# xuanvinh1997/llm-fp8

Hardware: AMD Instinct MI355X
Metric: train tokens/sec + FP8 GEMM % of MFMA peak, Llama-3.2-3B seq512 b16 (higher is better)
Workload: dtype fp8 (E4M3/E5M2 operands, fp32 accumulate, bf16 activations); 1 GPU; llama-3.2-3b (28 layers) full fine-tuning step, batch 16/GPU x seq 512, fp8_scenario=default (te_llama counterpart, lm_head FP8 under the outer recipe), random-init weights, synthetic tokens; route=fused, global_batch=16, seq_len=512, parallelism=single

## Files before the change

include/mi_fp8.h:

```cpp
#ifndef MI_FP8_H
#define MI_FP8_H

#include <stdint.h>

#ifdef __cplusplus
extern "C" {
#endif

#define MI_FMT_E4M3 0
#define MI_FMT_E5M2 1

#define MI_OK 0
#define MI_ERR_ARG (-1)
#define MI_ERR_SHAPE (-2)
#define MI_ERR_HIP (-3)

#define MI_OUT_BF16 0
#define MI_OUT_F32 1

#define MI_AMAX_ALGO_MAX 0
#define MI_AMAX_ALGO_MOST_RECENT 1

#define MI_ABI_VERSION 5
int mi_abi_version(void);
// ... 73 lines not shown

int mi_dswiglu_cast(const void* h_bf16, const void* dact_bf16, void* y_fp8, void* yT_fp8, const float* scale,
                    float* amax, float* colsum, int64_t rows, int64_t F, int fmt, void* stream);
int mi_swiglu_cast_bias(const void* h_bf16, const void* bias_bf16, void* y_fp8, void* yT_fp8, const float* scale, float* amax,
                        int64_t rows, int64_t F, int fmt, void* stream);
int mi_dswiglu_cast_bias(const void* h_bf16, const void* bias_bf16, const void* dact_bf16, void* y_fp8, void* yT_fp8,
                         const float* scale, float* amax, float* colsum, int64_t rows, int64_t F, int fmt, void* stream);

int mi_rmsnorm_stats(const void* x_bf16, float* rstd, int64_t rows, int64_t cols, float eps, void* stream);
int mi_add_rmsnorm_stats(const void* a_bf16, const void* b_bf16, void* out_bf16, float* rstd, int64_t rows, int64_t cols,
                         float eps, void* stream);
int mi_add_bias_rmsnorm_stats(const void* a_bf16, const void* b_bf16, const void* bias_bf16, void* out_bf16, float* rstd,
                              int64_t rows, int64_t cols, float eps, void* stream);
int mi_norm_cast(const void* x_bf16, const float* rstd, const void* gamma_bf16, void* y_fp8, void* yT_fp8,
                 const float* scale, float* amax, int64_t rows, int64_t cols, int fmt, void* stream);
int mi_rmsnorm_bwd(const void* dy_bf16, const void* x_bf16, const float* rstd, const void* gamma_bf16,
                   const void* dres_bf16, void* dx_bf16, float* dgamma_partial, int n_partials, int64_t rows,
                   int64_t cols, void* stream);

int mi_ce_forward(const void* logits_bf16, const int64_t* labels, float* lse, float* loss_rows, int64_t rows,
                  int64_t cols, void* stream);
int mi_ce_backward(const void* logits_bf16, const int64_t* labels, const float* lse, const float* gscale,
                   void* dlogits_bf16, int64_t rows, int64_t cols, void* stream);
int mi_ce_backward_cast(const void* logits_bf16, const int64_t* labels, const float* lse, const float* gscale, void* y_fp8,
                        void* yT_fp8, const float* scale, float* amax, int64_t rows, int64_t cols, int fmt, void* stream);

int mi_sumsq_bf16(const void* g_bf16, int64_t n, float* partial, int n_partials, void* stream);
int mi_sumsq_bf16_multi(const int64_t* table, int n_tensors, const int32_t* chunks, int n_chunks, int chunk_elems,
                        double* partial, void* stream);
int mi_adamw_bf16_multi(const int64_t* table, int n_tensors, const int32_t* chunks, int n_chunks, int chunk_elems,
// ... 31 lines not shown
```

llm_fp8_amd/_lib.py:

```python
from __future__ import annotations

import ctypes
import os

_HERE = os.path.dirname(os.path.abspath(__file__))
LIB_PATH = os.environ.get("LLM_FP8_AMD_LIB") or os.path.join(_HERE, "libmi_fp8.so")
LAB_LIB_PATH = os.path.join(os.path.dirname(_HERE), "tools", "bin", "libmi_fp8_lab.so")

MI_FMT_E4M3 = 0
MI_FMT_E5M2 = 1
ABI_VERSION = 5

_c_i64 = ctypes.c_int64
_c_int = ctypes.c_int
_p = ctypes.c_void_p

class GemmProblem(ctypes.Structure):
    _fields_ = [("A", ctypes.c_void_p), ("B", ctypes.c_void_p), ("D", ctypes.c_void_p), ("sa_inv", ctypes.c_void_p),
                ("sb_inv", ctypes.c_void_p), ("M", ctypes.c_int64), ("N", ctypes.c_int64), ("K", ctypes.c_int64),
                ("lda", ctypes.c_int64), ("ldb", ctypes.c_int64), ("ldd", ctypes.c_int64)]


class GemmMxProblem(ctypes.Structure):
    _fields_ = [("A", ctypes.c_void_p), ("SA", ctypes.c_void_p), ("B", ctypes.c_void_p), ("SB", ctypes.c_void_p),
# ... 38 lines not shown
    "mi_cast_amax_colsum": [_p, _p, _p, _p, _p, _p, _c_i64, _c_i64, _c_i64, _c_i64, _c_int, _p],
    "mi_colsum_finish": [_p, _c_i64, _c_i64, _p, _c_int, _p],
    "mi_colsum_finish_multi": [_p, _p, _p, _p, _p, _c_int, _p],
    "mi_gemm_workspace_bytes": [],
    "mi_gemm_set_workspace": [_p, _c_i64],
    "mi_attn_fwd": [_p, _p, _p, _p, _p, _c_int, _c_int, _c_int, _c_int, _c_int, _c_i64, _c_i64, _c_i64, _c_i64, ctypes.c_float,
                    _c_int, _p],
    "mi_attn_bwd": [_p] * 10 + [_c_int] * 5 + [_c_i64] * 8 + [ctypes.c_float, _c_int, _p],
    "mi_mxfp8_norm_quantize": [_p, _p, _p, _p, _p, _p, _p, _c_i64, _c_i64, _c_int, _p],
    "mi_mxfp8_swiglu_quantize": [_p, _p, _p, _p, _p, _c_i64, _c_i64, _c_int, _p],
    "mi_mxfp8_dswiglu_quantize": [_p, _p, _p, _p, _p, _p, _p, _c_i64, _c_i64, _c_int, _p],
    "mi_gemm_mxfp8": [_p, _p, _p, _p, _p, _p, _c_i64, _c_i64, _c_i64, _c_int, _c_int, _c_int, _c_int, _p],
    "mi_swiglu_cast_bias": [_p, _p, _p, _p, _p, _p, _c_i64, _c_i64, _c_int, _p],
    "mi_dswiglu_cast_bias": [_p, _p, _p, _p, _p, _p, _p, _p, _c_i64, _c_i64, _c_int, _p],
    "mi_add_bias_rmsnorm_stats": [_p, _p, _p, _p, _p, _c_i64, _c_i64, ctypes.c_float, _p],
    "mi_gemm_fp8_clock": [_p, _p, _p, _p, _p, _c_i64, _c_i64, _c_i64, _c_i64, _c_i64, _c_i64, _c_int, _p, _p],
}
LAB_SIGNATURES = {
    "mi_attn_fwd_diag": [_p, _p, _p, _p, _p, _p, _c_int, _c_int, _c_int, _c_int, _c_int, _c_i64, _c_i64, _c_i64, _c_i64, ctypes.c_float, _p],
}

_lib = None


def _bind(path: str, signatures) -> ctypes.CDLL:
    lib = ctypes.CDLL(path)
    for name, argtypes in signatures.items():
        fn = getattr(lib, name)
        fn.argtypes = argtypes
        fn.restype = ctypes.c_char_p if name == "mi_last_error" else (_c_i64 if name == "mi_gemm_workspace_bytes" else _c_int)
# ... 37 lines not shown
```

llm_fp8_amd/csrc/mi_fused.hip:

```cpp
#include "mi_common.h"

namespace mi {

template <int DIR>
__global__ __launch_bounds__(256) void rope_qkv_kernel(uint16_t* __restrict__ fused, uint16_t* __restrict__ q,
                                                       uint16_t* __restrict__ k, uint16_t* __restrict__ v,
                                                       const float* __restrict__ cosT, const float* __restrict__ sinT,
                                                       int rows, int seq, int nq, int nk, int D) {
  const int half = D >> 1;
  const int vph = half >> 3;
  const int W = (nq + 2 * nk) * D;
  const int rot_items = (nq + nk) * vph;
  const int cpy_items = (nk * D) >> 3;
  const int per_row = rot_items + cpy_items;
  const int64_t items = (int64_t)rows * per_row;
  const float sgn = DIR == 0 ? 1.0f : -1.0f;
  for (int64_t it = (int64_t)blockIdx.x * blockDim.x + threadIdx.x; it < items; it += (int64_t)gridDim.x * blockDim.x) {
    const int64_t r = it / per_row;
    const int w = (int)(it - r * per_row);
    uint16_t* frow = fused + r * W;
    if (w < rot_items) {
      const int hd = w / vph, vv = w - hd * vph;
      uint16_t* sep = hd < nq ? q + (r * nq + hd) * D : k + (r * nk + (hd - nq)) * D;
      uint16_t* f1 = frow + hd * D + vv * 8;
// ... 854 lines not shown
  const uint16_t *xp = (const uint16_t*)x_bf16, *gp = (const uint16_t*)gamma_bf16;
  uint8_t *yp = (uint8_t*)y_fp8, *tp = (uint8_t*)yT_fp8;
#define MI_NC(FMTv)                                                                                                        \
  if (y_fp8 && yT_fp8)                                                                                                     \
    hipLaunchKernelGGL((mi::norm_cast_kernel<FMTv, true, true>), grid, block, 0, st, xp, rstd, gp, yp, tp, scale, amax, (int)rows, (int)cols, tiles_c); \
  else if (y_fp8)                                                                                                          \
    hipLaunchKernelGGL((mi::norm_cast_kernel<FMTv, true, false>), grid, block, 0, st, xp, rstd, gp, yp, tp, scale, amax, (int)rows, (int)cols, tiles_c); \
  else                                                                                                                     \
    hipLaunchKernelGGL((mi::norm_cast_kernel<FMTv, false, true>), grid, block, 0, st, xp, rstd, gp, yp, tp, scale, amax, (int)rows, (int)cols, tiles_c);
  if (fmt == MI_FMT_E4M3) { MI_NC(MI_FMT_E4M3) } else { MI_NC(MI_FMT_E5M2) }
#undef MI_NC
  MI_CHECK_LAUNCH("mi_norm_cast launch");
  return MI_OK;
}

extern "C" int mi_rmsnorm_bwd(const void* dy_bf16, const void* x_bf16, const float* rstd, const void* gamma_bf16,
                              const void* dres_bf16, void* dx_bf16, float* dgamma_partial, int n_partials, int64_t rows,
                              int64_t cols, void* stream) {
  MI_CHECK_ARG(dy_bf16 && x_bf16 && rstd && gamma_bf16 && dx_bf16 && dgamma_partial, "mi_rmsnorm_bwd: null pointer");
  MI_CHECK_ARG(rows >= 0 && cols > 0 && cols % 512 == 0 && cols <= 512 * mi::kNormMaxVec, "mi_rmsnorm_bwd: cols must be a multiple of 512, at most %d", 512 * mi::kNormMaxVec);
  MI_CHECK_ARG(n_partials >= 1 && rows < (1LL << 31), "mi_rmsnorm_bwd: bad sizes");
  MI_CHECK_ARG(((uintptr_t)dy_bf16 % 16) == 0 && ((uintptr_t)x_bf16 % 16) == 0 && ((uintptr_t)gamma_bf16 % 16) == 0 &&
                   ((uintptr_t)dres_bf16 % 16) == 0 && ((uintptr_t)dx_bf16 % 16) == 0, "mi_rmsnorm_bwd: misaligned pointer");
  const int rows_per_block = (int)((rows + n_partials - 1) / n_partials);
  const int rpb = rows_per_block < 1 ? 1 : rows_per_block;
  const size_t shm = (size_t)(4 * cols * sizeof(float));
#define MI_RB(NV, WPRv)                                                                                                   \
  case NV:                                                                                                                \
    hipLaunchKernelGGL((mi::rmsnorm_bwd_kernel<NV, WPRv>), dim3(n_partials), dim3(256), shm, (hipStream_t)stream,         \
                       (const uint16_t*)dy_bf16, (const uint16_t*)x_bf16, rstd, (const uint16_t*)gamma_bf16,              \
// ... 67 lines not shown
```

llm_fp8_amd/llama.py:

```python
from __future__ import annotations

import os
import re
from contextlib import contextmanager
from typing import Dict, Optional

import torch

from . import pytorch as te
from .common.recipe import DelayedScaling, Format, MXFP8BlockScaling
from .pytorch.fp8 import FP8GlobalStateManager
from .pytorch.module import _can_fuse_norm, residual_add_stats

LLAMA_CONFIGS: Dict[str, dict] = {
    "llama-3.2-1b": dict(hidden_size=2048, intermediate_size=8192, num_hidden_layers=16, num_attention_heads=32,
                         num_key_value_heads=8, head_dim=64, tie_word_embeddings=True),
    "llama-3.2-3b": dict(hidden_size=3072, intermediate_size=8192, num_hidden_layers=28, num_attention_heads=24,
                         num_key_value_heads=8, head_dim=128, tie_word_embeddings=True),
    "llama-3.1-8b": dict(hidden_size=4096, intermediate_size=14336, num_hidden_layers=32, num_attention_heads=32,
                         num_key_value_heads=8, head_dim=128, tie_word_embeddings=False),
}
_ALIASES = {"meta-llama/llama-3.2-1b": "llama-3.2-1b", "meta-llama/llama-3.2-3b": "llama-3.2-3b",
            "meta-llama/llama-3.1-8b": "llama-3.1-8b", "meta-llama/meta-llama-3.1-8b": "llama-3.1-8b"}


def llama_config(name: str, **overrides):
    from transformers import LlamaConfig
# ... 26 lines not shown

_ROPE_CACHE: Dict[tuple, torch.Tensor] = {}


def _rope_table(dim: int, max_len: int, device) -> torch.Tensor:
    key = (dim, max_len, str(device))
    if key not in _ROPE_CACHE:
        _ROPE_CACHE[key] = te.attention.RotaryPositionEmbedding(dim)(max_seq_len=max_len).to(device)
    return _ROPE_CACHE[key]


def _handed_rstd(h: torch.Tensor):
    tag = getattr(h, "_mi_rstd", None)
    if tag is None or tag[2] != h._version:
        return None
    return tag[0], tag[1]


class TELlamaDecoderLayer(torch.nn.Module):

    scenario = "default"

    def __init__(self, config, *args, dropout_rate: float = 0.0, **kwargs):
        super().__init__()
        dev = "cuda" if torch.cuda.is_available() else "cpu"
        self.attn_recipe, self.mlp_recipe = scenario_recipes(self.scenario)
        self.self_attention = te.MultiheadAttention(
            hidden_size=config.hidden_size,
            num_attention_heads=config.num_attention_heads,
            kv_channels=getattr(config, "head_dim", None) or config.hidden_size // config.num_attention_heads,
            bias=False,
# ... 3 lines not shown
            normalization="RMSNorm",
            num_gqa_groups=config.num_key_value_heads,
            qkv_format="bshd",
            input_layernorm=True,
            device=dev,
        )
        self.layernorm_mlp = te.LayerNormMLP(
            hidden_size=config.hidden_size,
            ffn_hidden_size=config.intermediate_size,
            normalization="RMSNorm",
            activation="swiglu",
            device=dev,
        )
        head_dim = getattr(config, "head_dim", None) or config.hidden_size // config.num_attention_heads
        self.te_rope_emb = _rope_table(head_dim, config.max_position_embeddings, dev)

    route = "fused"

    def forward(self, hidden_states, attention_mask=None, **kwargs):
        if not isinstance(hidden_states, torch.Tensor):
            raise TypeError("hidden_states must be a torch.Tensor")
        if attention_mask is not None and not isinstance(attention_mask, torch.Tensor):
            raise TypeError("attention_mask must be a torch.Tensor")
        fp8 = hidden_states.is_cuda
        if self.route == "reference":
            with te.fp8_autocast(enabled=fp8, fp8_recipe=self.attn_recipe):
                hidden_states = hidden_states + self.self_attention(hidden_states, attention_mask=attention_mask,
                                                                    rotary_pos_emb=self.te_rope_emb)
            with te.fp8_autocast(enabled=fp8, fp8_recipe=self.mlp_recipe):
                hidden_states = hidden_states + self.layernorm_mlp(hidden_states)
            return hidden_states
        with te.fp8_autocast(enabled=fp8, fp8_recipe=self.attn_recipe):
            attn_out, skip = self.self_attention(hidden_states, attention_mask=attention_mask, rotary_pos_emb=self.te_rope_emb,
                                                 _with_skip=True, _rstd=_handed_rstd(hidden_states))
        eps_mlp = self.layernorm_mlp.eps
        hidden_states, rstd = residual_add_stats(skip, attn_out, eps_mlp)
        with te.fp8_autocast(enabled=fp8, fp8_recipe=self.mlp_recipe):
            ffn_out, skip, ffn_bias = self.layernorm_mlp(hidden_states, _with_skip=True, _rstd=(rstd, eps_mlp), _defer_bias=True)
        eps_in = self.self_attention.layernorm_qkv.eps
        hidden_states, rstd = residual_add_stats(skip, ffn_out, eps_in, bias=ffn_bias)
        if rstd is not None:
            hidden_states._mi_rstd = (rstd, eps_in, hidden_states._version)
        return hidden_states


def decoder_layer_cls(scenario: str):
    scenario_recipes(scenario)
    return type(f"TELlamaDecoderLayer_{scenario}", (TELlamaDecoderLayer,), {"scenario": scenario})


@contextmanager
def replace_decoder(te_decoder_cls):
    import transformers
    mod = transformers.models.llama.modeling_llama
    original = mod.LlamaDecoderLayer
    mod.LlamaDecoderLayer = te_decoder_cls
    try:
# ... 49 lines not shown

    model.forward = forward


class _FinalNormView:
    fused_norm, normalization, zero_centered_gamma = True, "RMSNorm", False


class TELlamaForCausalLM:

    def __new__(cls, config, scenario: str = "default"):
        from transformers.models.llama.modeling_llama import LlamaForCausalLM
        with replace_decoder(te_decoder_cls=decoder_layer_cls(scenario)):
            model = LlamaForCausalLM(config)
        model.model.register_forward_pre_hook(_drop_padding_mask, with_kwargs=True)
        _install_final_norm_fusion(model)
        return model

    @classmethod
    def from_pretrained_local(cls, pretrained_model_name_or_path, *args, config, scenario: str = "default",
                              torch_dtype=torch.bfloat16, **kwargs):
        from . import checkpoint
        prev = torch.get_default_dtype()
        torch.set_default_dtype(torch_dtype)
        try:
            model = cls(config, scenario)
        finally:
            torch.set_default_dtype(prev)
        checkpoint.load_into(model, str(pretrained_model_name_or_path), config)
        return model
# ... 122 lines not shown
```

llm_fp8_amd/pytorch/module.py:

```python
from __future__ import annotations

import io
import os
from typing import List, Optional, Sequence, Tuple

import torch
import torch.nn.functional as F

from ..common.recipe import DelayedScaling, Format, MXFP8BlockScaling, Recipe, fmt_codes
from . import ops
from .fp8 import FP8GlobalStateManager, ModuleMeta

__all__ = ["Linear", "LayerNormLinear", "LayerNormMLP", "LayerNorm", "RMSNorm"]


def _as_bf16_2d(t: torch.Tensor) -> torch.Tensor:
    t2 = t.reshape(-1, t.shape[-1])
    if t2.dtype != torch.bfloat16:
        t2 = t2.to(torch.bfloat16)
    return t2.contiguous()


class DyHandoff:
    __slots__ = ("scale", "amax", "fmt", "want_y", "want_t", "fp8", "ptr", "mx", "act_ref")
# ... 21 lines not shown
                               "(an op was inserted between the q|k|v projection and the rotary split)")
        fp8, self.fp8, self.ptr = self.fp8, None, None
        return fp8


def handoff_readers(t) -> bool:
    if torch.is_anomaly_enabled():
        return True
    if t is None:
        return False
    return bool(getattr(t, "retains_grad", False)) or bool(getattr(t, "_backward_hooks", None))


class _GemmSpec:
    __slots__ = ("recipe", "meta_fwd", "meta_bwd", "g", "fmt_fwd", "fmt_bwd", "trigger_bwd_update", "training", "eps",
                 "wcache", "first_mb", "with_skip", "rstd", "dy_handoff", "defer_bias", "q")

    def __init__(self, recipe, meta_fwd, meta_bwd, g, trigger_bwd_update, training, eps=1e-5, wcache=None, first_mb=None,
                 with_skip=False, rstd=None, dy_handoff=None, defer_bias=False):
        self.dy_handoff = dy_handoff
        self.defer_bias = defer_bias
        self.eps = eps
        self.rstd = rstd
        self.with_skip = with_skip
        self.wcache, self.first_mb = wcache, first_mb
        self.recipe, self.meta_fwd, self.meta_bwd, self.g = recipe, meta_fwd, meta_bwd, g
        self.fmt_fwd, self.fmt_bwd = fmt_codes(recipe.fp8_format)
        self.q = _MXQ(self.fmt_fwd, self.fmt_bwd) if recipe.mxfp8() else _DelayedQ(meta_fwd, meta_bwd, self.fmt_fwd, self.fmt_bwd)
        self.trigger_bwd_update = trigger_bwd_update
        self.training = training


class _Sink:
    __slots__ = ("parts", "stamp")

# ... 93 lines not shown
    no_sink = "row-sharded weights of this shape cannot take an FP8 sink"
    swiglu_adds_bias = True
    colsum_dtypes = None

    def __init__(self, mf, mb, fmt_f: int, fmt_b: int):
        self.mf, self.mb, self.fmt_f, self.fmt_b = mf, mb, fmt_f, fmt_b

    def _act(self, y, yT, s: int):
        return (y, self.mf.scale_inv(s)), (yT, self.mf.scale_inv_snapshot()[s:s + 1])

    def quantize(self, x2, g: int, want_t: bool, norm=None):
        mf, s = self.mf, 3 * g
        if norm is None:
            return self._act(*ops.cast_amax(x2, mf.scale(s), mf.amax(s), self.fmt_f, want_t=want_t), s)
        return self._act(*ops.norm_cast(x2, norm[0], norm[1], mf.scale(s), mf.amax(s), self.fmt_f, want_t=want_t), s)

    def swiglu(self, h, g: int, want_t: bool, bias):
        mf, s = self.mf, 3 * g
        return self._act(*ops.swiglu_cast(h, mf.scale(s), mf.amax(s), self.fmt_f, want_t=want_t, bias=bias), s)

    def _grad(self, y, yT, cs, s: int):
        si = self.mb.scale_inv(s)
        return (y, si), (yT, si), cs

    def quantize_grad(self, g2, g: int, want_y: bool, want_t: bool, colsum: bool = False):
        mb, s = self.mb, 2 * g
        out = ops.cast_amax(g2, mb.scale(s), mb.amax(s), self.fmt_b, want_y=want_y, want_t=want_t, want_colsum=colsum)
        return self._grad(out[0], out[1], out[2] if colsum else None, s)

    def dswiglu(self, h, dact, g: int, want_y: bool, want_t: bool, colsum: bool, bias):
# ... 165 lines not shown
    @staticmethod
    def backward(ctx, dout, _drstd):
        return dout, dout, None, None


def residual_add_stats(a: torch.Tensor, b: torch.Tensor, eps: float, bias: Optional[torch.Tensor] = None):
    if (a.is_cuda and a.dtype == torch.bfloat16 and b.dtype == torch.bfloat16 and a.shape == b.shape and a.is_contiguous()
            and b.is_contiguous() and a.shape[-1] % 8 == 0 and (bias is None or a.shape[-1] == bias.numel())):
        bb = None if bias is None else bias.detach().to(torch.bfloat16).contiguous()
        return _AddStatsFn.apply(a, b, eps, bb)
    if bias is not None:
        b = b + bias.detach().to(b.dtype)
    return a + b, None


def _wgrad_out(weights, K: int) -> Optional[torch.Tensor]:
    shard = getattr(weights[0], "_mi_sharded", None)
    if shard is not None:
        return shard.dp.wgrad_buffer(weights, K)
    slot = getattr(weights[0], "_mi_grad_slot", None)
    if slot is None:
        return None
    arena, off = slot
    if arena.dtype != torch.bfloat16:
        return None
    end = off
    for w in weights:
        s = getattr(w, "_mi_grad_slot", None)
        if s is None or s[0] is not arena or s[1] != end or w.grad is not None or w.dtype != torch.bfloat16 or w.shape[1] != K:
            return None
# ... 26 lines not shown
def _skip_2d(dskip: Optional[torch.Tensor], like: torch.Tensor) -> Optional[torch.Tensor]:
    if dskip is None:
        return None
    d = dskip.reshape(like.shape)
    return d if (d.dtype == torch.bfloat16 and d.is_contiguous()) else d.to(torch.bfloat16).contiguous()


def _quantize_input(ctx, spec: _GemmSpec, x2, ln_w, want_t: bool, need_dgrad: bool):
    ctx.norm = None
    if ln_w is None:
        return spec.q.quantize(x2, spec.g, want_t)
    gam = (ln_w if ln_w.dtype == torch.bfloat16 else ln_w.to(torch.bfloat16)).contiguous()
    rstd = spec.rstd if spec.rstd is not None else ops.rmsnorm_stats(x2, spec.eps)
    if need_dgrad:
        ctx.norm = (x2, rstd, gam, ln_w.dtype)
    return spec.q.quantize(x2, spec.g, want_t, (rstd, gam))


def _finish_dx(ctx, dx, dskip, colsums=None):
    dln = None
    if ctx.norm is not None and dx is not None:
        xin, rstd, gam, ln_dtype = ctx.norm
        ctx.norm = None
        dx, dln = ops.rmsnorm_bwd(dx, xin, rstd, gam, dres=_skip_2d(dskip, dx), dgamma_dtype=ln_dtype, finish=colsums is None)
        dskip = None
        if colsums is not None:
            dln = (dln, ln_dtype)
    if colsums is not None:
        pend = [t for t in (*colsums, dln) if t is not None]
        if pend:
# ... 298 lines not shown
        for n, sz in zip(self.bias_names, sizes):
            if bias:
                setattr(self, n, torch.nn.Parameter(torch.zeros(sz, dtype=dt, device=device)))
            else:
                setattr(self, n, None)

    def _weights(self):
        return [getattr(self, n) for n in self.weight_names]

    def _bias(self):
        if not self.use_bias:
            return None
        bs = [getattr(self, n) for n in self.bias_names]
        return bs[0] if len(bs) == 1 else torch.cat(bs, 0)

    def forward(self, inp: torch.Tensor, is_first_microbatch=None, _with_skip: bool = False, _rstd=None, _dy_handoff=None):
        st = self._prepare(inp.device)
        ws, b = self._weights(), self._bias()
        if st is not None and _can_fuse_norm(self, st[0], inp) and not self.return_layernorm_output:
            return _FP8LinearFn.apply(inp, b, self._spec(st, is_first_microbatch, eps=self.eps, with_skip=_with_skip,
                                                         rstd=_usable_rstd(_rstd, inp, self.eps), dy_handoff=_dy_handoff),
                                      self.layer_norm_weight, *ws)
        ln = self._norm(inp)
        if st is None:
            w = _master(ws[0]) if len(ws) == 1 else torch.cat([_master(w_) for w_ in ws], 0)
            out = F.linear(ln, w.to(ln.dtype), None if b is None else b.to(ln.dtype))
        else:
            out = _FP8LinearFn.apply(ln, b, self._spec(st, is_first_microbatch), None, *ws)
        if _with_skip:
            return out, inp
        return (out, ln) if self.return_layernorm_output else out


def _usable_rstd(handoff, inp: torch.Tensor, eps: float):
    if handoff is None:
        return None
    rstd, e = handoff
    if rstd is None or e != eps or rstd.numel() != inp.numel() // inp.shape[-1] or rstd.device != inp.device:
        return None
    return rstd


def _can_fuse_norm(mod, recipe, inp) -> bool:
    h = inp.shape[-1]
    return (getattr(mod, "fused_norm", True) and mod.normalization == "RMSNorm" and not mod.zero_centered_gamma
            and (recipe.delayed() or recipe.mxfp8()) and h % 512 == 0 and h // 512 in (1, 2, 3, 4, 5, 6, 7, 8, 10, 12, 14, 16))


def _swiglu(a: torch.Tensor) -> torch.Tensor:
    f = a.shape[-1] // 2
    return F.silu(a[..., :f]) * a[..., f:]


_ACTS = {
    "swiglu": (_swiglu, 2), "gelu": (lambda a: F.gelu(a, approximate="tanh"), 1), "relu": (F.relu, 1),
# ... 14 lines not shown
        self.hidden_size, self.ffn_hidden_size, self.eps = hidden_size, ffn_hidden_size, eps
        self.normalization, self.activation, self.zero_centered_gamma = normalization, activation, zero_centered_gamma
        self.act_fn, mult = _ACTS[activation]
        dt = params_dtype or torch.get_default_dtype()
        self.layer_norm_weight = torch.nn.Parameter(
            torch.zeros(hidden_size, dtype=dt, device=device) if zero_centered_gamma else torch.ones(hidden_size, dtype=dt, device=device))
        self.layer_norm_bias = (torch.nn.Parameter(torch.zeros(hidden_size, dtype=dt, device=device))
                                if normalization == "LayerNorm" else None)
        self.fc1_weight = _init_weight((mult * ffn_hidden_size, hidden_size), dt, device, init_method)
        self.fc2_weight = _init_weight((hidden_size, ffn_hidden_size), dt, device, output_layer_init_method or init_method)
        self.use_bias = bias
        self.fc1_bias = torch.nn.Parameter(torch.zeros(mult * ffn_hidden_size, dtype=dt, device=device)) if bias else None
        self.fc2_bias = torch.nn.Parameter(torch.zeros(hidden_size, dtype=dt, device=device)) if bias else None
        self.fused_swiglu = True

    def forward(self, inp: torch.Tensor, is_first_microbatch=None, _with_skip: bool = False, _rstd=None, _defer_bias: bool = False):
        st = self._prepare(inp.device)
        if (st is not None and self.activation == "swiglu" and self.fused_swiglu and _can_fuse_norm(self, st[0], inp)):
            defer = bool(_defer_bias and _with_skip and _FUSE_MLP_BIAS and self.fc2_bias is not None)
            res = _FP8SwiGLUMLPFn.apply(inp, self.fc1_weight, self.fc1_bias, self.fc2_weight, self.fc2_bias,
                                        self._spec(st, is_first_microbatch, eps=self.eps, with_skip=_with_skip,
                                                   rstd=_usable_rstd(_rstd, inp, self.eps), defer_bias=defer),
                                        self.layer_norm_weight)
            if _defer_bias and _with_skip:
                return res[0], res[1], (self.fc2_bias if defer else None)
            return res
        out = self._unfused(inp, st, is_first_microbatch)
        if _defer_bias and _with_skip:
            return out, inp, None
        return (out, inp) if _with_skip else out

    def _unfused(self, inp, st, is_first_microbatch):
        ln = self._norm(inp)
        if st is None:
            h = F.linear(ln, _master(self.fc1_weight).to(ln.dtype), None if self.fc1_bias is None else self.fc1_bias.to(ln.dtype))
            return F.linear(self.act_fn(h), _master(self.fc2_weight).to(ln.dtype),
                            None if self.fc2_bias is None else self.fc2_bias.to(ln.dtype))
# ... 7 lines not shown
```

llm_fp8_amd/pytorch/ops.py:

```python
from __future__ import annotations

import ctypes
import os
from typing import Optional, Tuple

import torch

from .. import _lib
from .profiler import KernelTimer

E4M3, E5M2 = _lib.MI_FMT_E4M3, _lib.MI_FMT_E5M2
FP8_MAX = {E4M3: 448.0, E5M2: 57344.0}


_SK_WORKSPACE = {}


def ensure_gemm_workspace(device: torch.device) -> None:
    idx = device.index if device.index is not None else torch.cuda.current_device()
    if idx in _SK_WORKSPACE:
        return
    lib = _lib.load()
    with torch.cuda.device(idx):
        nbytes = int(lib.mi_gemm_workspace_bytes())
# ... 575 lines not shown
    assert x.dtype == torch.bfloat16 and gamma.dtype == torch.bfloat16 and x.is_contiguous() and gamma.is_contiguous()
    R, C = x.shape
    y = torch.empty((R, C), dtype=torch.uint8, device=x.device) if want_y else None
    yT = torch.empty((C, R), dtype=torch.uint8, device=x.device) if want_t else None
    args = (x.data_ptr(), rstd.data_ptr(), gamma.data_ptr(), _ptr(y), _ptr(yT), scale.data_ptr(), _ptr(amax), R, C, fmt, _stream())
    t = KernelTimer.active
    if t is None:
        rc = _lib.load().mi_norm_cast(*args)
    else:
        with t.span("norm_cast", f"{R}x{C}", float(R * C), float(R * C * (2 + int(want_y) + int(want_t)))):
            rc = _lib.load().mi_norm_cast(*args)
    _lib.check(rc, "mi_norm_cast")
    return y, yT


def rmsnorm_bwd(dy: torch.Tensor, x: torch.Tensor, rstd: torch.Tensor, gamma: torch.Tensor,
                dres: Optional[torch.Tensor] = None, n_partials: int = 512, dgamma_dtype: torch.dtype = torch.float32,
                finish: bool = True):
    _dev(dy, x, rstd, gamma, dres)
    assert dy.dtype == torch.bfloat16 and x.dtype == torch.bfloat16 and dy.is_contiguous() and x.is_contiguous()
    R, C = x.shape
    n_partials = max(1, min(n_partials, (R + 3) // 4))
    dx = torch.empty_like(x)
    part = torch.empty((n_partials, C), dtype=torch.float32, device=x.device)
    rc = _lib.load().mi_rmsnorm_bwd(dy.data_ptr(), x.data_ptr(), rstd.data_ptr(), gamma.data_ptr(), _ptr(dres), dx.data_ptr(),
                                    part.data_ptr(), n_partials, R, C, _stream())
    _lib.check(rc, "mi_rmsnorm_bwd")
    return (dx, colsum_finish(part, dgamma_dtype)) if finish else (dx, part)


# ... 122 lines not shown
```

Baseline: 87250 tokens/s.

## Fuse residual add, RMSNorm statistics and FP8 cast into one kernel

Adds a HIP kernel that does the residual add (with optional bias), computes per-row RMSNorm rstd, and writes the normalized FP8 output and its transpose in a single pass. Each wave keeps 8 whole rows in registers. The decoder layers are linked so the cast for the next layer's QKV norm (and the MLP norm) happens at the residual add. The consumer module then reuses the precast when scale, weight version and shape still match. This removes a separate norm_cast kernel, so the residual is not re-read from memory for every norm. In exchange it brings in precast validity tracking and a kernel that only handles column counts of 2048, 3072 or 4096 and row counts that are multiples of 32.

```diff
diff --git a/include/mi_fp8.h b/include/mi_fp8.h
--- a/include/mi_fp8.h
+++ b/include/mi_fp8.h
@@ -111,6 +111,11 @@
                               int64_t rows, int64_t cols, float eps, void* stream);
 int mi_norm_cast(const void* x_bf16, const float* rstd, const void* gamma_bf16, void* y_fp8, void* yT_fp8,
                  const float* scale, float* amax, int64_t rows, int64_t cols, int fmt, void* stream);
+int mi_add_norm_cast(const void* a_bf16, const void* b_bf16, const void* gamma_bf16, void* out_bf16, float* rstd, void* y_fp8,
+                     void* yT_fp8, const float* scale, float* amax, int64_t rows, int64_t cols, float eps, int fmt, void* stream);
+int mi_add_bias_norm_cast(const void* a_bf16, const void* b_bf16, const void* bias_bf16, const void* gamma_bf16, void* out_bf16,
+                          float* rstd, void* y_fp8, void* yT_fp8, const float* scale, float* amax, int64_t rows, int64_t cols,
+                          float eps, int fmt, void* stream);
 int mi_rmsnorm_bwd(const void* dy_bf16, const void* x_bf16, const float* rstd, const void* gamma_bf16,
                    const void* dres_bf16, void* dx_bf16, float* dgamma_partial, int n_partials, int64_t rows,
                    int64_t cols, void* stream);
diff --git a/llm_fp8_amd/_lib.py b/llm_fp8_amd/_lib.py
--- a/llm_fp8_amd/_lib.py
+++ b/llm_fp8_amd/_lib.py
@@ -76,6 +76,8 @@
     "mi_swiglu_cast_bias": [_p, _p, _p, _p, _p, _p, _c_i64, _c_i64, _c_int, _p],
     "mi_dswiglu_cast_bias": [_p, _p, _p, _p, _p, _p, _p, _p, _c_i64, _c_i64, _c_int, _p],
     "mi_add_bias_rmsnorm_stats": [_p, _p, _p, _p, _p, _c_i64, _c_i64, ctypes.c_float, _p],
+    "mi_add_norm_cast": [_p, _p, _p, _p, _p, _p, _p, _p, _p, _c_i64, _c_i64, ctypes.c_float, _c_int, _p],
+    "mi_add_bias_norm_cast": [_p, _p, _p, _p, _p, _p, _p, _p, _p, _p, _c_i64, _c_i64, ctypes.c_float, _c_int, _p],
     "mi_gemm_fp8_clock": [_p, _p, _p, _p, _p, _c_i64, _c_i64, _c_i64, _c_i64, _c_i64, _c_i64, _c_int, _p, _p],
 }
 LAB_SIGNATURES = {
diff --git a/llm_fp8_amd/csrc/mi_fused.hip b/llm_fp8_amd/csrc/mi_fused.hip
--- a/llm_fp8_amd/csrc/mi_fused.hip
+++ b/llm_fp8_amd/csrc/mi_fused.hip
@@ -892,6 +892,203 @@
   return MI_OK;
 }
 
+namespace mi {
+template <int FMT, int NVEC, bool BIAS, bool WRITE_T>
+__global__ __launch_bounds__(256) void add_norm_cast_kernel(const uint16_t* __restrict__ a, const uint16_t* __restrict__ b,
+                                                            const uint16_t* __restrict__ bias, const uint16_t* __restrict__ gamma,
+                                                            uint16_t* __restrict__ out, float* __restrict__ rstd,
+                                                            uint8_t* __restrict__ y, uint8_t* __restrict__ yT,
+                                                            const float* __restrict__ scale_p, float* amax_out, int rows,
+                                                            int cols_rt, float eps) {
+  constexpr int cols = NVEC * 512;
+  __shared__ float s_amax[4];
+  const int tid = threadIdx.x, lane = tid & 63, wave = tid >> 6;
+  const int bands = rows >> 5, per_xcd = bands >> 3, id = blockIdx.x;
+  const int band = id < per_xcd * 8 ? (id & 7) * per_xcd + (id >> 3) : id;
+  const int r0 = band * 32 + wave * 8;
+  u32 s[8][NVEC][4];
+  float rs[8];
+  constexpr bool kAhead = NVEC < 8;
+  v4i gvs[NVEC], vbias[NVEC], na[NVEC], nb[NVEC];
+  const int64_t off0 = (int64_t)r0 * cols + lane * 8;
+  if (kAhead) {
+#pragma unroll
+    for (int k = 0; k < NVEC; ++k) {
+      na[k] = __builtin_nontemporal_load(reinterpret_cast<const v4i*>(a + off0 + k * 512));
+      nb[k] = __builtin_nontemporal_load(reinterpret_cast<const v4i*>(b + off0 + k * 512));
+    }
+#pragma unroll
+    for (int k = 0; k < NVEC; ++k) {
+      gvs[k] = *reinterpret_cast<const v4i*>(gamma + lane * 8 + k * 512);
+      if (BIAS) vbias[k] = *reinterpret_cast<const v4i*>(bias + lane * 8 + k * 512);
+    }
+  }
+#pragma unroll
+  for (int i = 0; i < 8; ++i) {
+    const int64_t off = off0 + (int64_t)i * cols;
+    v4i ca[NVEC], cb[NVEC];
+#pragma unroll
+    for (int k = 0; k < NVEC; ++k) {
+      if (kAhead) {
+        ca[k] = na[k];
+        cb[k] = nb[k];
+      } else {
+        ca[k] = __builtin_nontemporal_load(reinterpret_cast<const v4i*>(a + off + k * 512));
+        cb[k] = __builtin_nontemporal_load(reinterpret_cast<const v4i*>(b + off + k * 512));
+        if (BIAS) vbias[k] = *reinterpret_cast<const v4i*>(bias + lane * 8 + k * 512);
+      }
+    }
+    if (kAhead && i < 7) {
+#pragma unroll
+      for (int k = 0; k < NVEC; ++k) {
+        na[k] = __builtin_nontemporal_load(reinterpret_cast<const v4i*>(a + off + cols + k * 512));
+        nb[k] = __builtin_nontemporal_load(reinterpret_cast<const v4i*>(b + off + cols + k * 512));
+      }
+    }
+    __builtin_amdgcn_sched_barrier(0);
+    float acc = 0.0f;
+#pragma unroll
+    for (int k = 0; k < NVEC; ++k) {
+      const v4i va = ca[k], vb = cb[k];
+      v4i vo;
+#pragma unroll
+      for (int j = 0; j < 4; ++j) {
+        const u32 wa = (u32)va[j], wb = (u32)vb[j];
+        float b0 = __uint_as_float(wb << 16), b1 = __uint_as_float(wb & 0xFFFF0000u);
+        if (BIAS) {
+          b0 += __uint_as_float((u32)vbias[k][j] << 16);
+          b1 += __uint_as_float((u32)vbias[k][j] & 0xFFFF0000u);
+        }
+        const u32 o = pack_bf16x2(__uint_as_float(wa << 16) + b0, __uint_as_float(wa & 0xFFFF0000u) + b1);
+        const float lo = __uint_as_float(o << 16), hi = __uint_as_float(o & 0xFFFF0000u);
+        acc += lo * lo + hi * hi;
+        vo[j] = (int)o;
+        s[i][k][j] = o;
+        asm volatile("" : "+v"(s[i][k][j]));
+      }
+      *reinterpret_cast<v4i*>(out + off + k * 512) = vo;
+      __builtin_amdgcn_sched_barrier(0);
+    }
+#pragma unroll
+    for (int o = 32; o >= 1; o >>= 1) acc += __shfl_xor(acc, o);
+    rs[i] = rsqrtf(acc / (float)cols_rt + eps);
+    if (lane == 0) rstd[r0 + i] = rs[i];
+    __builtin_amdgcn_sched_barrier(0);
+  }
+  const float scale = *scale_p;
+  float amax = 0.0f;
+#pragma unroll
+  for (int k = 0; k < NVEC; ++k) {
+    const int c0 = k * 512 + lane * 8;
+    const v4i gv = kAhead ? gvs[k] : *reinterpret_cast<const v4i*>(gamma + c0);
+    float g[8];
+#pragma unroll
+    for (int j = 0; j < 4; ++j) {
+      g[2 * j] = __uint_as_float((u32)gv[j] << 16);
+      g[2 * j + 1] = __uint_as_float((u32)gv[j] & 0xFFFF0000u);
+    }
+    u32 lo[8], hi[8];
+#pragma unroll
+    for (int i = 0; i < 8; ++i) {
+      float f[8];
+#pragma unroll
+      for (int j = 0; j < 4; ++j) {
+        const u32 w = s[i][k][j];
+        f[2 * j] = (__uint_as_float(w << 16) * rs[i]) * g[2 * j];
+        f[2 * j + 1] = (__uint_as_float(w & 0xFFFF0000u) * rs[i]) * g[2 * j + 1];
+      }
+#pragma unroll
+      for (int j = 0; j < 8; ++j) amax = fmaxf(amax, (f[j] != f[j]) ? 0.0f : fabsf(f[j]));
+      lo[i] = cvt4_fp8<FMT>(f[0] * scale, f[1] * scale, f[2] * scale, f[3] * scale);
+      hi[i] = cvt4_fp8<FMT>(f[4] * scale, f[5] * scale, f[6] * scale, f[7] * scale);
+    }
+    uint8_t* dst = y + (int64_t)r0 * cols + c0;
+#pragma unroll
+    for (int i = 0; i < 8; ++i) mi::st8<MI_NT_Y>(dst + (int64_t)i * cols, lo[i], hi[i]);
+    if (WRITE_T) {
+      u32 ta[4], tb[4], tc[4], td[4];
+      transpose4x4(lo[0], lo[1], lo[2], lo[3], ta[0], ta[1], ta[2], ta[3]);
+      transpose4x4(lo[4], lo[5], lo[6], lo[7], tb[0], tb[1], tb[2], tb[3]);
+      transpose4x4(hi[0], hi[1], hi[2], hi[3], tc[0], tc[1], tc[2], tc[3]);
+      transpose4x4(hi[4], hi[5], hi[6], hi[7], td[0], td[1], td[2], td[3]);
+      uint8_t* dt = yT + (int64_t)c0 * rows + r0;
+#pragma unroll
+      for (int j = 0; j < 4; ++j) {
+        mi::st8<MI_NT_YT>(dt + (int64_t)j * rows, ta[j], tb[j]);
+        mi::st8<MI_NT_YT>(dt + (int64_t)(j + 4) * rows, tc[j], td[j]);
+      }
+    }
+    __builtin_amdgcn_sched_barrier(0);
+  }
+  if (amax_out != nullptr) {
+    amax = wave_max(amax);
+    if (lane == 0) s_amax[wave] = amax;
+    __syncthreads();
+    if (tid == 0) {
+      float m = fmaxf(fmaxf(s_amax[0], s_amax[1]), fmaxf(s_amax[2], s_amax[3]));
+      if (m > 0.0f && m > __builtin_nontemporal_load(amax_out)) atomicMax(reinterpret_cast<unsigned int*>(amax_out), __float_as_uint(m));
+    }
+  }
+}
+
+template <int FMT, int NVEC>
+static void launch_add_norm_cast(const void* a, const void* b, const void* bias, const void* gamma, void* out, float* rstd, void* y,
+                                 void* yT, const float* scale, float* amax, int64_t rows, float eps, hipStream_t st) {
+  dim3 grid((unsigned)(rows / 32)), block(256);
+  const uint16_t *ap = (const uint16_t*)a, *bp = (const uint16_t*)b, *sp = (const uint16_t*)bias, *gp = (const uint16_t*)gamma;
+  uint16_t* op = (uint16_t*)out;
+  uint8_t *yp = (uint8_t*)y, *tp = (uint8_t*)yT;
+  const int cols = NVEC * 512;
+#define MI_ANC(BIASv, Tv) \
+  hipLaunchKernelGGL((add_norm_cast_kernel<FMT, NVEC, BIASv, Tv>), grid, block, 0, st, ap, bp, sp, gp, op, rstd, yp, tp, scale, amax, (int)rows, cols, eps)
+  if (bias != nullptr) {
+    if (yT != nullptr) MI_ANC(true, true); else MI_ANC(true, false);
+  } else {
+    if (yT != nullptr) MI_ANC(false, true); else MI_ANC(false, false);
+  }
+#undef MI_ANC
+}
+
+static int add_norm_cast_host(const char* who, const void* a, const void* b, const void* bias, bool with_bias, const void* gamma,
+                              void* out, float* rstd, void* y, void* yT, const float* scale, float* amax, int64_t rows,
+                              int64_t cols, float eps, int fmt, void* stream) {
+  MI_CHECK_ARG(a && b && gamma && out && rstd && y && scale && (!with_bias || bias), "%s: null pointer", who);
+  MI_CHECK_ARG(fmt == MI_FMT_E4M3 || fmt == MI_FMT_E5M2, "%s: bad fmt %d", who, fmt);
+  MI_CHECK_ARG(rows >= 0 && rows % 32 == 0 && rows < (1LL << 31), "%s: rows must be a multiple of 32 (a workgroup owns a band of 32 rows), got %lld",
+               who, (long long)rows);
+  MI_CHECK_ARG(cols == 2048 || cols == 3072 || cols == 4096,
+               "%s: cols must be 2048, 3072 or 4096 (a wave keeps 8 whole rows in registers), got %lld", who, (long long)cols);
+  MI_CHECK_ARG((((uintptr_t)a | (uintptr_t)b | (uintptr_t)out | (uintptr_t)gamma | (uintptr_t)bias | (uintptr_t)rstd) % 16) == 0 &&
+                   (((uintptr_t)y | (uintptr_t)yT) % 8) == 0, "%s: misaligned pointer", who);
+  if (rows == 0) return MI_OK;
+  hipStream_t st = (hipStream_t)stream;
+#define MI_ANC_W(FMTv)                                                                                                    \
+  switch (cols) {                                                                                                         \
+    case 2048: launch_add_norm_cast<FMTv, 4>(a, b, bias, gamma, out, rstd, y, yT, scale, amax, rows, eps, st); break;      \
+    case 3072: launch_add_norm_cast<FMTv, 6>(a, b, bias, gamma, out, rstd, y, yT, scale, amax, rows, eps, st); break;      \
+    default: launch_add_norm_cast<FMTv, 8>(a, b, bias, gamma, out, rstd, y, yT, scale, amax, rows, eps, st); break;        \
+  }
+  if (fmt == MI_FMT_E4M3) { MI_ANC_W(MI_FMT_E4M3) } else { MI_ANC_W(MI_FMT_E5M2) }
+#undef MI_ANC_W
+  MI_CHECK_LAUNCH(who);
+  return MI_OK;
+}
+}
+
+extern "C" int mi_add_norm_cast(const void* a_bf16, const void* b_bf16, const void* gamma_bf16, void* out_bf16, float* rstd,
+                                void* y_fp8, void* yT_fp8, const float* scale, float* amax, int64_t rows, int64_t cols, float eps,
+                                int fmt, void* stream) {
+  return mi::add_norm_cast_host("mi_add_norm_cast", a_bf16, b_bf16, nullptr, false, gamma_bf16, out_bf16, rstd, y_fp8, yT_fp8, scale,
+                                amax, rows, cols, eps, fmt, stream);
+}
+
+extern "C" int mi_add_bias_norm_cast(const void* a_bf16, const void* b_bf16, const void* bias_bf16, const void* gamma_bf16,
+                                     void* out_bf16, float* rstd, void* y_fp8, void* yT_fp8, const float* scale, float* amax,
+                                     int64_t rows, int64_t cols, float eps, int fmt, void* stream) {
+  return mi::add_norm_cast_host("mi_add_bias_norm_cast", a_bf16, b_bf16, bias_bf16, true, gamma_bf16, out_bf16, rstd, y_fp8, yT_fp8,
+                                scale, amax, rows, cols, eps, fmt, stream);
+}
+
 extern "C" int mi_rmsnorm_bwd(const void* dy_bf16, const void* x_bf16, const float* rstd, const void* gamma_bf16,
                               const void* dres_bf16, void* dx_bf16, float* dgamma_partial, int n_partials, int64_t rows,
                               int64_t cols, void* stream) {
diff --git a/llm_fp8_amd/llama.py b/llm_fp8_amd/llama.py
--- a/llm_fp8_amd/llama.py
+++ b/llm_fp8_amd/llama.py
@@ -10,7 +10,7 @@
 from . import pytorch as te
 from .common.recipe import DelayedScaling, Format, MXFP8BlockScaling
 from .pytorch.fp8 import FP8GlobalStateManager
-from .pytorch.module import _can_fuse_norm, residual_add_stats
+from .pytorch.module import _can_fuse_norm, residual_add_norm_cast
 
 LLAMA_CONFIGS: Dict[str, dict] = {
     "llama-3.2-1b": dict(hidden_size=2048, intermediate_size=8192, num_hidden_layers=16, num_attention_heads=32,
@@ -67,7 +67,14 @@
     tag = getattr(h, "_mi_rstd", None)
     if tag is None or tag[2] != h._version:
         return None
-    return tag[0], tag[1]
+    return tag[0], tag[1], (tag[3] if len(tag) > 3 else None)
+
+
+def link_decoder_layers(layers) -> None:
+    layers = list(layers)
+    for cur, nxt in zip(layers, layers[1:] + [None]):
+        if isinstance(cur, TELlamaDecoderLayer):
+            cur._mi_next = (nxt if isinstance(nxt, TELlamaDecoderLayer) else None,)
 
 
 class TELlamaDecoderLayer(torch.nn.Module):
@@ -101,6 +108,7 @@
         )
         head_dim = getattr(config, "head_dim", None) or config.hidden_size // config.num_attention_heads
         self.te_rope_emb = _rope_table(head_dim, config.max_position_embeddings, dev)
+        self._mi_next = (None,)
 
     route = "fused"
 
@@ -121,13 +129,18 @@
             attn_out, skip = self.self_attention(hidden_states, attention_mask=attention_mask, rotary_pos_emb=self.te_rope_emb,
                                                  _with_skip=True, _rstd=_handed_rstd(hidden_states))
         eps_mlp = self.layernorm_mlp.eps
-        hidden_states, rstd = residual_add_stats(skip, attn_out, eps_mlp)
+        hidden_states, rstd, pc = residual_add_norm_cast(skip, attn_out, eps_mlp, None, self.layernorm_mlp, self.mlp_recipe if fp8 else None)
         with te.fp8_autocast(enabled=fp8, fp8_recipe=self.mlp_recipe):
-            ffn_out, skip, ffn_bias = self.layernorm_mlp(hidden_states, _with_skip=True, _rstd=(rstd, eps_mlp), _defer_bias=True)
+            ffn_out, skip, ffn_bias = self.layernorm_mlp(hidden_states, _with_skip=True, _rstd=(rstd, eps_mlp, pc), _defer_bias=True)
         eps_in = self.self_attention.layernorm_qkv.eps
-        hidden_states, rstd = residual_add_stats(skip, ffn_out, eps_in, bias=ffn_bias)
+        nxt = self._mi_next[0]
+        if nxt is not None and nxt.route == "fused" and nxt.self_attention.layernorm_qkv.eps == eps_in:
+            hidden_states, rstd, pc = residual_add_norm_cast(skip, ffn_out, eps_in, ffn_bias, nxt.self_attention.layernorm_qkv,
+                                                             nxt.attn_recipe if fp8 else None)
+        else:
+            hidden_states, rstd, pc = residual_add_norm_cast(skip, ffn_out, eps_in, ffn_bias)
         if rstd is not None:
-            hidden_states._mi_rstd = (rstd, eps_in, hidden_states._version)
+            hidden_states._mi_rstd = (rstd, eps_in, hidden_states._version, pc)
         return hidden_states
 
 
@@ -207,6 +220,7 @@
         with replace_decoder(te_decoder_cls=decoder_layer_cls(scenario)):
             model = LlamaForCausalLM(config)
         model.model.register_forward_pre_hook(_drop_padding_mask, with_kwargs=True)
+        link_decoder_layers(model.model.layers)
         _install_final_norm_fusion(model)
         return model
 
diff --git a/llm_fp8_amd/pytorch/module.py b/llm_fp8_amd/pytorch/module.py
--- a/llm_fp8_amd/pytorch/module.py
+++ b/llm_fp8_amd/pytorch/module.py
@@ -59,11 +59,12 @@
 
 class _GemmSpec:
     __slots__ = ("recipe", "meta_fwd", "meta_bwd", "g", "fmt_fwd", "fmt_bwd", "trigger_bwd_update", "training", "eps",
-                 "wcache", "first_mb", "with_skip", "rstd", "dy_handoff", "defer_bias", "q")
+                 "wcache", "first_mb", "with_skip", "rstd", "dy_handoff", "defer_bias", "q", "precast")
 
     def __init__(self, recipe, meta_fwd, meta_bwd, g, trigger_bwd_update, training, eps=1e-5, wcache=None, first_mb=None,
-                 with_skip=False, rstd=None, dy_handoff=None, defer_bias=False):
+                 with_skip=False, rstd=None, dy_handoff=None, defer_bias=False, precast=None):
         self.dy_handoff = dy_handoff
+        self.precast = precast
         self.defer_bias = defer_bias
         self.eps = eps
         self.rstd = rstd
@@ -187,6 +188,9 @@
         if norm is None:
             return self._act(*ops.cast_amax(x2, mf.scale(s), mf.amax(s), self.fmt_f, want_t=want_t), s)
         return self._act(*ops.norm_cast(x2, norm[0], norm[1], mf.scale(s), mf.amax(s), self.fmt_f, want_t=want_t), s)
+
+    def ahead(self, pc, g: int, want_t: bool):
+        return self._act(pc.y, pc.yT if want_t else None, 3 * g)
 
     def swiglu(self, h, g: int, want_t: bool, bias):
         mf, s = self.mf, 3 * g
@@ -382,6 +386,66 @@
     return a + b, None
 
 
+class _PreCast:
+    __slots__ = ("ptr", "shape", "version", "rstd", "ln_w", "ln_version", "arena", "generation", "scale_ptr", "fmt", "y", "yT")
+
+    def fits(self, x2, rstd, ln_w, spec, want_t: bool) -> bool:
+        q = spec.q
+        if q.mx or spec.g != 0:
+            return False
+        return (x2.data_ptr() == self.ptr and tuple(x2.shape) == self.shape and x2._version == self.version and rstd is self.rstd
+                and ln_w is self.ln_w and ln_w._version == self.ln_version and q.mf.arena is self.arena
+                and self.arena.generation == self.generation and q.mf.scale(0).data_ptr() == self.scale_ptr and q.fmt_f == self.fmt
+                and (self.yT is not None or not want_t))
+
+
+class _AddNormCastFn(_AddStatsFn):
+
+    @staticmethod
+    def forward(ctx, a, b, eps, bias, gamma, scale, amax, fmt, want_t, pc):
+        out, rstd, pc.y, pc.yT = ops.add_norm_cast(a, b, eps, gamma, scale, amax, fmt, bias=bias, want_t=want_t)
+        pc.rstd = rstd
+        ctx.mark_non_differentiable(rstd)
+        ctx.set_materialize_grads(False)
+        return out, rstd
+
+    @staticmethod
+    def backward(ctx, dout, _drstd):
+        return (dout, dout) + (None,) * 8
+
+
+def _ahead_plan(mod, recipe, like: torch.Tensor):
+    if os.environ.get("LLM_FP8_AMD_NO_ADD_NORM_FUSION") == "1" or mod is None or recipe is None or not recipe.delayed():
+        return None
+    if not _can_fuse_norm(mod, recipe, like) or not mod._takes_fused_norm():
+        return None
+    mf, ln_w = mod._meta_fwd, mod.layer_norm_weight
+    key = (recipe.fp8_format, recipe.amax_history_len, recipe.amax_compute_algo, recipe.margin, str(like.device))
+    if mf is None or mod._meta_key != key or ln_w.dtype != torch.bfloat16 or not ln_w.is_contiguous() or ln_w.data_ptr() % 16:
+        return None
+    want_t = torch.is_grad_enabled() and any(w.requires_grad for w in mod._gemm0_weights())
+    return ln_w, mf, fmt_codes(recipe.fp8_format)[0], want_t
+
+
+def residual_add_norm_cast(a: torch.Tensor, b: torch.Tensor, eps: float, bias: Optional[torch.Tensor] = None, consumer=None,
+                           recipe=None):
+    plan = None
+    if (a.is_cuda and a.dtype == torch.bfloat16 and b.dtype == torch.bfloat16 and a.shape == b.shape and a.is_contiguous()
+            and b.is_contiguous() and ops.add_norm_cast_ok(a.numel() // a.shape[-1], a.shape[-1])
+            and (bias is None or a.shape[-1] == bias.numel())):
+        plan = _ahead_plan(consumer, recipe, a)
+    if plan is None:
+        return residual_add_stats(a, b, eps, bias) + (None,)
+    ln_w, mf, fmt, want_t = plan
+    bb = None if bias is None else bias.detach().to(torch.bfloat16).contiguous()
+    pc = _PreCast()
+    out, rstd = _AddNormCastFn.apply(a, b, eps, bb, ln_w.detach(), mf.scale(0), mf.amax(0), fmt, want_t, pc)
+    pc.ptr, pc.shape, pc.version = out.data_ptr(), (out.numel() // out.shape[-1], out.shape[-1]), out._version
+    pc.ln_w, pc.ln_version = ln_w, ln_w._version
+    pc.arena, pc.generation, pc.scale_ptr, pc.fmt = mf.arena, mf.arena.generation, mf.scale(0).data_ptr(), fmt
+    return out, rstd, pc
+
+
 def _wgrad_out(weights, K: int) -> Optional[torch.Tensor]:
     shard = getattr(weights[0], "_mi_sharded", None)
     if shard is not None:
@@ -438,6 +502,8 @@
     rstd = spec.rstd if spec.rstd is not None else ops.rmsnorm_stats(x2, spec.eps)
     if need_dgrad:
         ctx.norm = (x2, rstd, gam, ln_w.dtype)
+    if spec.precast is not None and spec.precast.fits(x2, rstd, ln_w, spec, want_t):
+        return spec.q.ahead(spec.precast, spec.g, want_t)
     return spec.q.quantize(x2, spec.g, want_t, (rstd, gam))
 
 
@@ -766,12 +832,19 @@
         bs = [getattr(self, n) for n in self.bias_names]
         return bs[0] if len(bs) == 1 else torch.cat(bs, 0)
 
+    def _takes_fused_norm(self) -> bool:
+        return not self.return_layernorm_output
+
+    def _gemm0_weights(self):
+        return self._weights()
+
     def forward(self, inp: torch.Tensor, is_first_microbatch=None, _with_skip: bool = False, _rstd=None, _dy_handoff=None):
         st = self._prepare(inp.device)
         ws, b = self._weights(), self._bias()
-        if st is not None and _can_fuse_norm(self, st[0], inp) and not self.return_layernorm_output:
-            return _FP8LinearFn.apply(inp, b, self._spec(st, is_first_microbatch, eps=self.eps, with_skip=_with_skip,
-                                                         rstd=_usable_rstd(_rstd, inp, self.eps), dy_handoff=_dy_handoff),
+        if st is not None and _can_fuse_norm(self, st[0], inp) and self._takes_fused_norm():
+            rstd = _usable_rstd(_rstd, inp, self.eps)
+            return _FP8LinearFn.apply(inp, b, self._spec(st, is_first_microbatch, eps=self.eps, with_skip=_with_skip, rstd=rstd,
+                                                         dy_handoff=_dy_handoff, precast=_handed_precast(_rstd, rstd)),
                                       self.layer_norm_weight, *ws)
         ln = self._norm(inp)
         if st is None:
@@ -787,10 +860,14 @@
 def _usable_rstd(handoff, inp: torch.Tensor, eps: float):
     if handoff is None:
         return None
-    rstd, e = handoff
+    rstd, e = handoff[0], handoff[1]
     if rstd is None or e != eps or rstd.numel() != inp.numel() // inp.shape[-1] or rstd.device != inp.device:
         return None
     return rstd
+
+
+def _handed_precast(handoff, rstd):
+    return handoff[2] if (rstd is not None and handoff is not None and len(handoff) > 2) else None
 
 
 def _can_fuse_norm(mod, recipe, inp) -> bool:
@@ -835,13 +912,20 @@
         self.fc2_bias = torch.nn.Parameter(torch.zeros(hidden_size, dtype=dt, device=device)) if bias else None
         self.fused_swiglu = True
 
+    def _takes_fused_norm(self) -> bool:
+        return self.activation == "swiglu" and self.fused_swiglu
+
+    def _gemm0_weights(self):
+        return (self.fc1_weight, self.fc2_weight)
+
     def forward(self, inp: torch.Tensor, is_first_microbatch=None, _with_skip: bool = False, _rstd=None, _defer_bias: bool = False):
         st = self._prepare(inp.device)
-        if (st is not None and self.activation == "swiglu" and self.fused_swiglu and _can_fuse_norm(self, st[0], inp)):
+        if st is not None and self._takes_fused_norm() and _can_fuse_norm(self, st[0], inp):
             defer = bool(_defer_bias and _with_skip and _FUSE_MLP_BIAS and self.fc2_bias is not None)
+            rstd = _usable_rstd(_rstd, inp, self.eps)
             res = _FP8SwiGLUMLPFn.apply(inp, self.fc1_weight, self.fc1_bias, self.fc2_weight, self.fc2_bias,
-                                        self._spec(st, is_first_microbatch, eps=self.eps, with_skip=_with_skip,
-                                                   rstd=_usable_rstd(_rstd, inp, self.eps), defer_bias=defer),
+                                        self._spec(st, is_first_microbatch, eps=self.eps, with_skip=_with_skip, rstd=rstd,
+                                                   defer_bias=defer, precast=_handed_precast(_rstd, rstd)),
                                         self.layer_norm_weight)
             if _defer_bias and _with_skip:
                 return res[0], res[1], (self.fc2_bias if defer else None)
diff --git a/llm_fp8_amd/pytorch/ops.py b/llm_fp8_amd/pytorch/ops.py
--- a/llm_fp8_amd/pytorch/ops.py
+++ b/llm_fp8_amd/pytorch/ops.py
@@ -613,6 +613,41 @@
     return y, yT
 
 
+def add_norm_cast_ok(rows: int, cols: int) -> bool:
+    return rows > 0 and rows % 32 == 0 and cols in (2048, 3072, 4096)
+
+
+def add_norm_cast(a: torch.Tensor, b: torch.Tensor, eps: float, gamma: torch.Tensor, scale: torch.Tensor,
+                  amax: Optional[torch.Tensor], fmt: int, bias: Optional[torch.Tensor] = None, want_t: bool = True):
+    _dev(a, b, gamma, scale, amax, bias)
+    assert a.dtype == torch.bfloat16 and b.dtype == torch.bfloat16 and a.shape == b.shape and a.is_contiguous() and b.is_contiguous()
+    assert gamma.dtype == torch.bfloat16 and gamma.is_contiguous()
+    C = a.shape[-1]
+    R = a.numel() // C
+    if not add_norm_cast_ok(R, C):
+        return None
+    assert gamma.numel() == C
+    out = torch.empty_like(a)
+    rstd = torch.empty(R, dtype=torch.float32, device=a.device)
+    y = torch.empty((R, C), dtype=torch.uint8, device=a.device)
+    yT = torch.empty((C, R), dtype=torch.uint8, device=a.device) if want_t else None
+    tail = (gamma.data_ptr(), out.data_ptr(), rstd.data_ptr(), y.data_ptr(), _ptr(yT), scale.data_ptr(), _ptr(amax), R, C, float(eps),
+            fmt, _stream())
+    if bias is None:
+        fn, args = _lib.load().mi_add_norm_cast, (a.data_ptr(), b.data_ptr()) + tail
+    else:
+        assert bias.dtype == torch.bfloat16 and bias.numel() == C and bias.is_contiguous()
+        fn, args = _lib.load().mi_add_bias_norm_cast, (a.data_ptr(), b.data_ptr(), bias.data_ptr()) + tail
+    t = KernelTimer.active
+    if t is None:
+        rc = fn(*args)
+    else:
+        with t.span("norm_cast", f"{R}x{C}", float(R * C), float(R * C * (7 + int(want_t)))):
+            rc = fn(*args)
+    _lib.check(rc, "mi_add_norm_cast")
+    return out, rstd, y, yT
+
+
 def rmsnorm_bwd(dy: torch.Tensor, x: torch.Tensor, rstd: torch.Tensor, gamma: torch.Tensor,
                 dres: Optional[torch.Tensor] = None, n_partials: int = 512, dgamma_dtype: torch.dtype = torch.float32,
                 finish: bool = True):
```

Result: no change. 86720 tokens/s (-0.6%).
